# debbiemarkslab/EVcouplings

Measured on NVIDIA H100. Metric: PLM gradient evals/s as N*L^2*q cell-ops/s, higher is better.
Workload: dtype f32 parameters/accumulation; tensor-core products as bf16 hi+lo pairs (16 mantissa bits)

## Files before the change

evcouplings_b200/csrc/plm_tc.cu:

```cuda
#include <cuda.h>
#include <cuda_bf16.h>

#include <stdlib.h>

#include <algorithm>

#include "common.cuh"
#include "internal.h"

namespace evc {

constexpr int TC_BM = 128;
constexpr int TC_BN = 192;
constexpr int TC_BK = 64;
constexpr int TC_MAX_STAGES = 8;
constexpr int TC_A_BYTES = TC_BM * TC_BK * 2;
constexpr int TC_B_BYTES = TC_BN * TC_BK * 2;
constexpr int TC_SMEM_LIMIT = 232448;
constexpr int TC_SMEM_HEAD = 2048;
constexpr int TC_THREADS = 384;
constexpr int TC_CONSUMERS = 256;
constexpr int TC_K_CHUNK = 32;
constexpr int TC_MAX_KSPLIT = 8;
constexpr int TC_REG_PRODUCER = 40;
constexpr int TC_REG_CONSUMER = 232;

__device__ __forceinline__ void mbar_wait_bounded(uint64_t *bar, uint32_t parity)
{
    uint32_t done = 0;
    for (uint64_t it = 0; it < (1ull << 31); it++) {
        asm volatile(
            "{\n.reg .pred p;\n"
            "mbarrier.try_wait.parity.shared::cta.b64 p, [%1], %2;\n"
            "selp.u32 %0, 1, 0, p;\n}\n"
            : "=r"(done)
            : "r"(smem_u32(bar)), "r"(parity)
            : "memory");
        if (done) return;
    }
    __trap();
}

__device__ __forceinline__ void mbar_arrive(uint64_t *bar)
{
    asm volatile("mbarrier.arrive.shared::cta.b64 _, [%0];" ::"r"(smem_u32(bar)) : "memory");
}

__device__ __forceinline__ void tma_load_2d(void *smem_dst, const CUtensorMap *tmap, int c0, int c1, uint64_t *bar)
{
    asm volatile(
        "cp.async.bulk.tensor.2d.shared::cluster.global.mbarrier::complete_tx::bytes [%0], [%1, {%3, %4}], [%2];"
        ::"r"(smem_u32(smem_dst)), "l"(reinterpret_cast<uint64_t>(tmap)), "r"(smem_u32(bar)), "r"(c0), "r"(c1)
        : "memory");
}

__device__ __forceinline__ void tma_load_2d_hint(void *smem_dst, const CUtensorMap *tmap, int c0, int c1,
                                                 uint64_t *bar, uint64_t policy)
{
    asm volatile(
        "cp.async.bulk.tensor.2d.shared::cluster.global.mbarrier::complete_tx::bytes.L2::cache_hint "
        "[%0], [%1, {%3, %4}], [%2], %5;"
        ::"r"(smem_u32(smem_dst)), "l"(reinterpret_cast<uint64_t>(tmap)), "r"(smem_u32(bar)), "r"(c0), "r"(c1),
        "l"(policy)
        : "memory");
}
__device__ __forceinline__ uint64_t l2_policy_evict_last()
{
    uint64_t p;
    asm volatile("createpolicy.fractional.L2::evict_last.b64 %0, 1.0;" : "=l"(p));
    return p;
}

template <int N>
__device__ __forceinline__ void setmaxnreg_dec() { asm volatile("setmaxnreg.dec.sync.aligned.u32 %0;\n" ::"n"(N)); }
template <int N>
__device__ __forceinline__ void setmaxnreg_inc() { asm volatile("setmaxnreg.inc.sync.aligned.u32 %0;\n" ::"n"(N)); }

__device__ __forceinline__ void wgmma_fence() { asm volatile("wgmma.fence.sync.aligned;" ::: "memory"); }
__device__ __forceinline__ void wgmma_commit() { asm volatile("wgmma.commit_group.sync.aligned;" ::: "memory"); }
template <int N>
__device__ __forceinline__ void wgmma_wait() { asm volatile("wgmma.wait_group.sync.aligned %0;" ::"n"(N) : "memory"); }

template <int R>
__device__ __forceinline__ void fence_regs(float *d)
{
#pragma unroll
    for (int i = 0; i < R; i++) asm volatile("" : "+f"(d[i])::"memory");
}

__device__ __forceinline__ void consumer_sync() { asm volatile("bar.sync 1, %0;" ::"n"(TC_CONSUMERS) : "memory"); }

__device__ __forceinline__ uint64_t make_desc_sw128(const void *smem_ptr)
{
    const uint32_t addr = smem_u32(smem_ptr);
    uint64_t d = 0;
    d |= (uint64_t)((addr >> 4) & 0x3FFF);
    d |= (uint64_t)1 << 16;
    d |= (uint64_t)(1024 >> 4) << 32;
    d |= (uint64_t)1 << 62;
    return d;
}

template <int N>
__device__ __forceinline__ void wgmma_bf16(float *d, uint64_t da, uint64_t db, uint32_t scale_d);
template <>
__device__ __forceinline__ void wgmma_bf16<192>(float *d, uint64_t da, uint64_t db, uint32_t scale_d)
{
    asm volatile(
        "{\n.reg .pred p;\n"
        "setp.ne.b32 p, %98, 0;\n"
        "wgmma.mma_async.sync.aligned.m64n192k16.f32.bf16.bf16 "
        "{"
        "%0, %1, %2, %3, %4, %5, %6, %7, %8, %9, %10, %11, %12, %13, %14, %15, "
        "%16, %17, %18, %19, %20, %21, %22, %23, %24, %25, %26, %27, %28, %29, %30, %31, "
        "%32, %33, %34, %35, %36, %37, %38, %39, %40, %41, %42, %43, %44, %45, %46, %47, "
        "%48, %49, %50, %51, %52, %53, %54, %55, %56, %57, %58, %59, %60, %61, %62, %63, "
        "%64, %65, %66, %67, %68, %69, %70, %71, %72, %73, %74, %75, %76, %77, %78, %79, "
        "%80, %81, %82, %83, %84, %85, %86, %87, %88, %89, %90, %91, %92, %93, %94, %95"
        "}, %96, %97, p, 1, 1, 0, 0;\n}\n"
        : "+f"(d[0]), "+f"(d[1]), "+f"(d[2]), "+f"(d[3]), "+f"(d[4]), "+f"(d[5]), "+f"(d[6]), "+f"(d[7]),
          "+f"(d[8]), "+f"(d[9]), "+f"(d[10]), "+f"(d[11]), "+f"(d[12]), "+f"(d[13]), "+f"(d[14]), "+f"(d[15]),
          "+f"(d[16]), "+f"(d[17]), "+f"(d[18]), "+f"(d[19]), "+f"(d[20]), "+f"(d[21]), "+f"(d[22]), "+f"(d[23]),
          "+f"(d[24]), "+f"(d[25]), "+f"(d[26]), "+f"(d[27]), "+f"(d[28]), "+f"(d[29]), "+f"(d[30]), "+f"(d[31]),
          "+f"(d[32]), "+f"(d[33]), "+f"(d[34]), "+f"(d[35]), "+f"(d[36]), "+f"(d[37]), "+f"(d[38]), "+f"(d[39]),
          "+f"(d[40]), "+f"(d[41]), "+f"(d[42]), "+f"(d[43]), "+f"(d[44]), "+f"(d[45]), "+f"(d[46]), "+f"(d[47]),
          "+f"(d[48]), "+f"(d[49]), "+f"(d[50]), "+f"(d[51]), "+f"(d[52]), "+f"(d[53]), "+f"(d[54]), "+f"(d[55]),
          "+f"(d[56]), "+f"(d[57]), "+f"(d[58]), "+f"(d[59]), "+f"(d[60]), "+f"(d[61]), "+f"(d[62]), "+f"(d[63]),
          "+f"(d[64]), "+f"(d[65]), "+f"(d[66]), "+f"(d[67]), "+f"(d[68]), "+f"(d[69]), "+f"(d[70]), "+f"(d[71]),
          "+f"(d[72]), "+f"(d[73]), "+f"(d[74]), "+f"(d[75]), "+f"(d[76]), "+f"(d[77]), "+f"(d[78]), "+f"(d[79]),
          "+f"(d[80]), "+f"(d[81]), "+f"(d[82]), "+f"(d[83]), "+f"(d[84]), "+f"(d[85]), "+f"(d[86]), "+f"(d[87]),
          "+f"(d[88]), "+f"(d[89]), "+f"(d[90]), "+f"(d[91]), "+f"(d[92]), "+f"(d[93]), "+f"(d[94]), "+f"(d[95])
        : "l"(da), "l"(db), "r"(scale_d));
}
template <>
__device__ __forceinline__ void wgmma_bf16<176>(float *d, uint64_t da, uint64_t db, uint32_t scale_d)
{
    asm volatile(
        "{\n.reg .pred p;\n"
        "setp.ne.b32 p, %90, 0;\n"
        "wgmma.mma_async.sync.aligned.m64n176k16.f32.bf16.bf16 "
        "{"
        "%0, %1, %2, %3, %4, %5, %6, %7, %8, %9, %10, %11, %12, %13, %14, %15, "
        "%16, %17, %18, %19, %20, %21, %22, %23, %24, %25, %26, %27, %28, %29, %30, %31, "
        "%32, %33, %34, %35, %36, %37, %38, %39, %40, %41, %42, %43, %44, %45, %46, %47, "
        "%48, %49, %50, %51, %52, %53, %54, %55, %56, %57, %58, %59, %60, %61, %62, %63, "
        "%64, %65, %66, %67, %68, %69, %70, %71, %72, %73, %74, %75, %76, %77, %78, %79, "
        "%80, %81, %82, %83, %84, %85, %86, %87"
        "}, %88, %89, p, 1, 1, 0, 0;\n}\n"
        : "+f"(d[0]), "+f"(d[1]), "+f"(d[2]), "+f"(d[3]), "+f"(d[4]), "+f"(d[5]), "+f"(d[6]), "+f"(d[7]),
          "+f"(d[8]), "+f"(d[9]), "+f"(d[10]), "+f"(d[11]), "+f"(d[12]), "+f"(d[13]), "+f"(d[14]), "+f"(d[15]),
          "+f"(d[16]), "+f"(d[17]), "+f"(d[18]), "+f"(d[19]), "+f"(d[20]), "+f"(d[21]), "+f"(d[22]), "+f"(d[23]),
          "+f"(d[24]), "+f"(d[25]), "+f"(d[26]), "+f"(d[27]), "+f"(d[28]), "+f"(d[29]), "+f"(d[30]), "+f"(d[31]),
          "+f"(d[32]), "+f"(d[33]), "+f"(d[34]), "+f"(d[35]), "+f"(d[36]), "+f"(d[37]), "+f"(d[38]), "+f"(d[39]),
          "+f"(d[40]), "+f"(d[41]), "+f"(d[42]), "+f"(d[43]), "+f"(d[44]), "+f"(d[45]), "+f"(d[46]), "+f"(d[47]),
          "+f"(d[48]), "+f"(d[49]), "+f"(d[50]), "+f"(d[51]), "+f"(d[52]), "+f"(d[53]), "+f"(d[54]), "+f"(d[55]),
          "+f"(d[56]), "+f"(d[57]), "+f"(d[58]), "+f"(d[59]), "+f"(d[60]), "+f"(d[61]), "+f"(d[62]), "+f"(d[63]),
          "+f"(d[64]), "+f"(d[65]), "+f"(d[66]), "+f"(d[67]), "+f"(d[68]), "+f"(d[69]), "+f"(d[70]), "+f"(d[71]),
          "+f"(d[72]), "+f"(d[73]), "+f"(d[74]), "+f"(d[75]), "+f"(d[76]), "+f"(d[77]), "+f"(d[78]), "+f"(d[79]),
          "+f"(d[80]), "+f"(d[81]), "+f"(d[82]), "+f"(d[83]), "+f"(d[84]), "+f"(d[85]), "+f"(d[86]), "+f"(d[87])
        : "l"(da), "l"(db), "r"(scale_d));
}

__device__ __forceinline__ void wgmma_sp_bf16_192(float *d, const uint4 &a, uint32_t e, uint64_t db, uint32_t scale_d)
{
    asm volatile(
        "{\n.reg .pred p;\n"
        "setp.ne.b32 p, %102, 0;\n"
        "wgmma.mma_async.sp.sync.aligned.m64n192k32.f32.bf16.bf16 "
        "{"
        "%0, %1, %2, %3, %4, %5, %6, %7, %8, %9, %10, %11, %12, %13, %14, %15, "
        "%16, %17, %18, %19, %20, %21, %22, %23, %24, %25, %26, %27, %28, %29, %30, %31, "
        "%32, %33, %34, %35, %36, %37, %38, %39, %40, %41, %42, %43, %44, %45, %46, %47, "
        "%48, %49, %50, %51, %52, %53, %54, %55, %56, %57, %58, %59, %60, %61, %62, %63, "
        "%64, %65, %66, %67, %68, %69, %70, %71, %72, %73, %74, %75, %76, %77, %78, %79, "
        "%80, %81, %82, %83, %84, %85, %86, %87, %88, %89, %90, %91, %92, %93, %94, %95"
        "}, {%96, %97, %98, %99}, %100, %101, 0, p, 1, 1, 0;\n}\n"
        : "+f"(d[0]), "+f"(d[1]), "+f"(d[2]), "+f"(d[3]), "+f"(d[4]), "+f"(d[5]), "+f"(d[6]), "+f"(d[7]),
          "+f"(d[8]), "+f"(d[9]), "+f"(d[10]), "+f"(d[11]), "+f"(d[12]), "+f"(d[13]), "+f"(d[14]), "+f"(d[15]),
// ... 54 lines not shown
                                             bool overwrite)
{
#pragma unroll
    for (int k = 0; k < TC_BK / 16; k++) {
        const uint64_t koff = (uint64_t)((k * 16 * 2) >> 4);
        wgmma_bf16<N>(acc, a + koff, b + koff, (overwrite && k == 0) ? 0u : 1u);
        if (two) wgmma_bf16<N>(acc, a2 + koff, b2 + koff, 1u);
    }
}

template <int N>
__device__ __forceinline__ void tc_mainloop(float *acc, uint64_t *full, uint64_t *empty, int &s, uint32_t &ph,
                                            int n_stages, int stage_bytes, int kb0, int kb1, uint64_t desc0,
                                            uint64_t off_a, uint64_t off_b, uint64_t off_a2, uint64_t off_b2, bool two)
{
    int prev = -1;
    for (int kb = kb0; kb < kb1; kb++) {
        mbar_wait_bounded(&full[s], ph);
        wgmma_fence();
        const uint64_t d = desc0 + (uint64_t)((s * stage_bytes) >> 4);
        wgmma_kblock<N>(acc, d + off_a, d + off_b, d + off_a2, d + off_b2, two, kb == kb0);
        wgmma_commit();
        wgmma_wait<1>();
        if (prev >= 0) mbar_arrive(&empty[prev]);
        prev = s;
        if (++s == n_stages) { s = 0; ph ^= 1u; }
    }
    wgmma_wait<0>();
    fence_regs<N / 2>(acc);
    if (prev >= 0) mbar_arrive(&empty[prev]);
}

__device__ __forceinline__ void decode_tile(int tile, int m_tiles, int n_tiles, int mgroup, int &m_tile, int &n_tile)
{
    const int full = (m_tiles / mgroup) * mgroup * n_tiles;
    if (tile < full) {
        const int per = mgroup * n_tiles;
        const int g = tile / per, r = tile - g * per;
        n_tile = r / mgroup;
        m_tile = g * mgroup + (r - n_tile * mgroup);
    } else {
        const int rem = m_tiles % mgroup, r = tile - full;
        n_tile = r / rem;
        m_tile = (m_tiles / mgroup) * mgroup + (r - n_tile * rem);
    }
}

struct TcSmem {
    uint64_t *full, *empty;
    unsigned char *ring;
};
__device__ __forceinline__ TcSmem tc_smem_layout(unsigned char *smem_dyn)
{
    unsigned char *base = reinterpret_cast<unsigned char *>((reinterpret_cast<uintptr_t>(smem_dyn) + 1023) &
                                                            ~static_cast<uintptr_t>(1023));
    TcSmem l;
    l.full = reinterpret_cast<uint64_t *>(base);
    l.empty = l.full + TC_MAX_STAGES;
    l.ring = base + 1024;
    return l;
}
__device__ __forceinline__ void tc_init_barriers(const TcSmem &l, int n_stages)
{
    if (threadIdx.x == 0) {
        for (int s = 0; s < n_stages; s++) {
            mbar_init(&l.full[s], 1);
            mbar_init(&l.empty[s], TC_CONSUMERS);
        }
        mbar_fence_init();
    }
    __syncthreads();
}

template <int SINGLE, int ACC = 0>
__global__ void __launch_bounds__(TC_THREADS, 1)
tc_gemm_kernel(const __grid_constant__ CUtensorMap tm0, const __grid_constant__ CUtensorMap tm1,
               const __grid_constant__ CUtensorMap tm2, float *__restrict__ D, int64_t ldd, int m_tiles, int n_tiles,
               int num_kb, int k_chunk, int mgroup, int n_stages, int ksplit, int64_t plane, int acc_planes)
{
    constexpr int BYTES0 = TC_A_BYTES;
    constexpr int BYTES1 = TC_B_BYTES;
    constexpr int BYTES2 = TC_B_BYTES;
    constexpr int stage_bytes = BYTES0 + BYTES1 + (SINGLE ? 0 : BYTES2);
    extern __shared__ unsigned char smem_dyn[];
    const TcSmem l = tc_smem_layout(smem_dyn);
    const int tiles = m_tiles * n_tiles;
    const int slice = (int)blockIdx.x / tiles;
    int m_tile, n_tile;
    decode_tile((int)blockIdx.x - slice * tiles, m_tiles, n_tiles, mgroup, m_tile, n_tile);
    const int kb_per = (num_kb + ksplit - 1) / ksplit;
    const int kb_begin = slice * kb_per, kb_end = min(num_kb, kb_begin + kb_per);
    tc_init_barriers(l, n_stages);

    if (threadIdx.x < 128) {
        setmaxnreg_dec<TC_REG_PRODUCER>();
        if (threadIdx.x == 0) {
            int s = 0;
            uint32_t ph = 0;
            for (int kb = kb_begin; kb < kb_end; kb++) {
                mbar_wait_bounded(&l.empty[s], ph ^ 1u);
                unsigned char *st = l.ring + s * stage_bytes;
                mbar_expect_tx(&l.full[s], (uint32_t)stage_bytes);
                tma_load_2d(st, &tm0, kb * TC_BK, m_tile * TC_BM, &l.full[s]);
                tma_load_2d(st + BYTES0, &tm1, kb * TC_BK, n_tile * TC_BN, &l.full[s]);
                if (!SINGLE) tma_load_2d(st + BYTES0 + BYTES1, &tm2, kb * TC_BK, n_tile * TC_BN, &l.full[s]);
                if (++s == n_stages) { s = 0; ph ^= 1u; }
            }
        }
    } else {
        setmaxnreg_inc<TC_REG_CONSUMER>();
        const int cw = (threadIdx.x >> 7) - 1;
        constexpr uint64_t OFF1 = (uint64_t)(BYTES0 >> 4), OFF2 = (uint64_t)((BYTES0 + BYTES1) >> 4);
        const uint64_t arow = (uint64_t)((cw * 64 * TC_BK * 2) >> 4);
        const uint64_t desc0 = make_desc_sw128(l.ring);
        float acc[TC_BN / 2], sum[TC_BN / 2];
#pragma unroll
        for (int u = 0; u < TC_BN / 2; u++) acc[u] = 0.f;
        const int n_chunks = (kb_end - kb_begin + k_chunk - 1) / k_chunk;
        int s = 0;
        uint32_t ph = 0;
        for (int c = 0; c < n_chunks; c++) {
            const int kb0 = kb_begin + c * k_chunk, kb1 = min(kb_end, kb0 + k_chunk);
            tc_mainloop<TC_BN>(acc, l.full, l.empty, s, ph, n_stages, stage_bytes, kb0, kb1, desc0,
                               arow, OFF1, arow, OFF2, !SINGLE);
#pragma unroll
            for (int u = 0; u < TC_BN / 2; u++) sum[u] = (c == 0) ? acc[u] : sum[u] + acc[u];
        }
        const int t = threadIdx.x & 127;
        const int64_t row = (int64_t)m_tile * TC_BM + cw * 64 + (t >> 5) * 16 + ((t & 31) >> 2);
        float *out = D + slice * plane + row * ldd + (int64_t)n_tile * TC_BN + 2 * (t & 3);
        if (ACC && slice < acc_planes) {
#pragma unroll
            for (int c8 = 0; c8 < TC_BN / 8; c8++) {
                float2 *p0 = reinterpret_cast<float2 *>(out + 8 * c8);
                float2 *p1 = reinterpret_cast<float2 *>(out + 8 * ldd + 8 * c8);
                const float2 v0 = __ldcs(p0), v1 = __ldcs(p1);
                __stcs(p0, make_float2(v0.x + sum[4 * c8], v0.y + sum[4 * c8 + 1]));
                __stcs(p1, make_float2(v1.x + sum[4 * c8 + 2], v1.y + sum[4 * c8 + 3]));
            }
            return;
        }
#pragma unroll
        for (int c8 = 0; c8 < TC_BN / 8; c8++) {
            __stcs(reinterpret_cast<float2 *>(out + 8 * c8), make_float2(sum[4 * c8], sum[4 * c8 + 1]));
            __stcs(reinterpret_cast<float2 *>(out + 8 * ldd + 8 * c8), make_float2(sum[4 * c8 + 2], sum[4 * c8 + 3]));
        }
    }
}

constexpr int XSP_STEP_BYTES = 2560;
constexpr int XSP_KB_BYTES = 4 * XSP_STEP_BYTES;
constexpr int SP_W_HALF = (TC_BN / 2) * TC_BK * 2;

template <int SINGLE>
__global__ void __launch_bounds__(TC_THREADS, 1)
tc_sparse_logits_kernel(const __grid_constant__ CUtensorMap tm_hi, const __grid_constant__ CUtensorMap tm_lo,
                        const unsigned char *__restrict__ xsp, float *__restrict__ Zt, int64_t ldz, int64_t rows_z,
                        int state_tiles, int seq_tiles, int seq_units, int num_kb, int k_chunk, int group,
                        int n_stages)
{
    constexpr int OFF_A = TC_B_BYTES;
    constexpr int OFF_LO = TC_B_BYTES + XSP_KB_BYTES;
    constexpr int stage_bytes = OFF_LO + (SINGLE ? 0 : TC_B_BYTES);
    extern __shared__ unsigned char smem_dyn[];
    const TcSmem l = tc_smem_layout(smem_dyn);
    uint32_t cs;
    asm volatile("mov.u32 %0, %%cluster_nctarank;" : "=r"(cs));
    const uint32_t rank = cluster_ctarank();
    int n_tile, unit;
    decode_tile((int)(blockIdx.x / cs), state_tiles, seq_units, group, n_tile, unit);
    const int seq_tile = unit * (int)cs + (int)rank;
    const bool pad = seq_tile >= seq_tiles;
    if (threadIdx.x == 0) {
        for (int s = 0; s < n_stages; s++) {
            mbar_init(&l.full[s], 1);
            mbar_init(&l.empty[s], 8 * cs);
        }
        mbar_fence_init();
    }
    cluster_sync();

    if (threadIdx.x < 128) {
        setmaxnreg_dec<TC_REG_PRODUCER>();
        if (threadIdx.x == 0) {
            const uint64_t keep = l2_policy_evict_last();
            const unsigned char *src = xsp + (int64_t)(pad ? 0 : seq_tile) * num_kb * XSP_KB_BYTES;
            const int row0 = n_tile * TC_BN;
            int s = 0;
            uint32_t ph = 0;
            for (int kb = 0; kb < num_kb; kb++) {
                mbar_wait_bounded(&l.empty[s], ph ^ 1u);
                unsigned char *st = l.ring + s * stage_bytes;
                mbar_expect_tx(&l.full[s], (uint32_t)stage_bytes);
                bulk_g2s(st + OFF_A, src + (int64_t)kb * XSP_KB_BYTES, XSP_KB_BYTES, &l.full[s]);
                if (cs == 1) {
                    for (int h = 0; h < 2; h++) {
                        tma_load_2d_hint(st + h * SP_W_HALF, &tm_hi, kb * TC_BK, row0 + h * (TC_BN / 2), &l.full[s], keep);
                        if (!SINGLE)
                            tma_load_2d_hint(st + OFF_LO + h * SP_W_HALF, &tm_lo, kb * TC_BK, row0 + h * (TC_BN / 2),
                                             &l.full[s], keep);
                    }
                } else {
                    const int h = (int)rank;
                    tma_load_2d_multicast(st + h * SP_W_HALF, &tm_hi, kb * TC_BK, row0 + h * (TC_BN / 2), &l.full[s],
                                          (uint16_t)0x3, keep);
                    if (!SINGLE)
                        tma_load_2d_multicast(st + OFF_LO + h * SP_W_HALF, &tm_lo, kb * TC_BK, row0 + h * (TC_BN / 2),
                                              &l.full[s], (uint16_t)0x3, keep);
                }
                if (++s == n_stages) { s = 0; ph ^= 1u; }
            }
        }
    } else {
        setmaxnreg_inc<TC_REG_CONSUMER>();
        const int cw = (threadIdx.x >> 7) - 1;
        const int t = threadIdx.x & 127;
        const uint32_t a_addr = smem_u32(l.ring) + OFF_A + cw * 2 * XSP_STEP_BYTES + 16 * t;
        const uint32_t e_addr = a_addr + 2048 - 12 * t;
        const uint64_t desc0 = make_desc_sw128(l.ring);
        constexpr uint64_t DLO = (uint64_t)(OFF_LO >> 4), DK32 = (uint64_t)((32 * 2) >> 4);
        auto release = [&](int st) {
            if ((threadIdx.x & 31) == 0) {
                mbar_arrive_cluster(&l.empty[st], 0);
                if (cs == 2) mbar_arrive_cluster(&l.empty[st], 1);
            }
        };
        float acc[TC_BN / 2], sum[TC_BN / 2];
#pragma unroll
        for (int u = 0; u < TC_BN / 2; u++) acc[u] = 0.f;
        const int n_chunks = (num_kb + k_chunk - 1) / k_chunk;
        int s = 0;
        uint32_t ph = 0;
        for (int c = 0; c < n_chunks; c++) {
            const int kb0 = c * k_chunk, kb1 = min(num_kb, kb0 + k_chunk);
            for (int kb = kb0; kb < kb1; kb++) {
                mbar_wait_bounded(&l.full[s], ph);
                const uint32_t so = (uint32_t)(s * stage_bytes);
                const uint4 a0 = lds128(a_addr + so), a1 = lds128(a_addr + so + XSP_STEP_BYTES);
                const uint32_t e0 = lds32(e_addr + so), e1 = lds32(e_addr + so + XSP_STEP_BYTES);
                wgmma_fence();
                const uint64_t d = desc0 + (uint64_t)((s * stage_bytes) >> 4);
                wgmma_sp_bf16_192(acc, a0, e0, d, kb == kb0 ? 0u : 1u);
                if (!SINGLE) wgmma_sp_bf16_192(acc, a0, e0, d + DLO, 1u);
                wgmma_sp_bf16_192(acc, a1, e1, d + DK32, 1u);
                if (!SINGLE) wgmma_sp_bf16_192(acc, a1, e1, d + DLO + DK32, 1u);
                wgmma_commit();
                wgmma_wait<0>();
                release(s);
                if (++s == n_stages) { s = 0; ph ^= 1u; }
            }
            fence_regs<TC_BN / 2>(acc);
#pragma unroll
            for (int u = 0; u < TC_BN / 2; u++) sum[u] = (c == 0) ? acc[u] : sum[u] + acc[u];
        }
        if (!pad) {
            const int64_t seq0 = (int64_t)seq_tile * TC_BM + cw * 64 + (t >> 5) * 16 + ((t & 31) >> 2);
            const int64_t st0 = (int64_t)n_tile * TC_BN + 2 * (t & 3);
#pragma unroll
            for (int c8 = 0; c8 < TC_BN / 8; c8++)
#pragma unroll
                for (int e = 0; e < 4; e++) {
                    const int64_t row = st0 + 8 * c8 + (e & 1), col = seq0 + 8 * (e >> 1);
                    if (row < rows_z && col < ldz) __stcs(Zt + row * ldz + col, sum[4 * c8 + e]);
                }
        }
    }
    cluster_sync();
}

__device__ __forceinline__ uint32_t xsp_group(const uint32_t *__restrict__ msa4, int64_t Nld, int64_t n, bool real,
                                              int k, int lq, int q, uint32_t &vals)
{
    uint32_t mask = 0;
    if (real) {
#pragma unroll
        for (int p = 0; p < 4; p++) {
            const int kk = k + p;
            if (kk >= lq) break;
            const int j = kk / q, b = kk - j * q;
            const int code = (int)((msa4[(int64_t)(j >> 2) * Nld + n] >> (8 * (j & 3))) & 0xffu);
            mask |= (uint32_t)(code == b) << p;
        }
    }
    int i0 = 0, i1 = 1;
    if (__popc(mask) == 2) { i0 = __ffs(mask) - 1; i1 = 31 - __clz(mask); }
    else if (mask > 2) i1 = __ffs(mask) - 1;
    vals = (((mask >> i0) & 1u) ? 0x3F80u : 0u) | ((((mask >> i1) & 1u) ? 0x3F80u : 0u) << 16);
    return (uint32_t)(i0 | (i1 << 2));
}

__global__ void build_xsp_kernel(const uint32_t *__restrict__ msa4, unsigned char *__restrict__ out, int64_t n0,
                                 int64_t nreal, int64_t Nld, int L, int q, int num_kb, int64_t n_frag)
{
    const int64_t gt = (int64_t)blockIdx.x * blockDim.x + threadIdx.x;
    if (gt >= n_frag * 128) return;
    const int64_t ci = gt >> 7;
    const int t = (int)(gt & 127);
    const int step = (int)(ci & 1), cw = (int)((ci >> 1) & 1);
    const int64_t tkb = ci >> 2;
    const int kb = (int)(tkb % num_kb);
    const int64_t T = tkb / num_kb;
    const int64_t r0 = T * TC_BM + cw * 64 + (t >> 5) * 16 + ((t & 31) >> 2), r1 = r0 + 8;
    const int k0 = kb * TC_BK + step * 32, lq = L * q;
    const int c = t & 3, h = c & 1;
    uint32_t e = 0, v[2][2], unused;
#pragma unroll
    for (int rr = 0; rr < 2; rr++) {
        const int64_t r = rr ? r1 : r0;
#pragma unroll
        for (int i = 0; i < 4; i++)
            e |= xsp_group(msa4, Nld, n0 + r, r < nreal, k0 + 4 * (4 * h + i), lq, q, unused) << (16 * rr + 4 * i);
#pragma unroll
        for (int u = 0; u < 2; u++) xsp_group(msa4, Nld, n0 + r, r < nreal, k0 + 4 * (4 * u + c), lq, q, v[rr][u]);
    }
    unsigned char *frag = out + ci * XSP_STEP_BYTES;
    reinterpret_cast<uint4 *>(frag)[t] = make_uint4(v[0][0], v[1][0], v[0][1], v[1][1]);
    reinterpret_cast<uint32_t *>(frag + 2048)[t] = e;
}

constexpr int TF_BN = 176;
constexpr int TF_SITES = 8;
constexpr int TF_B_BYTES = TF_BN * TC_BK * 2;
constexpr int TF_PITCH = TF_BN + 1;

template <int SINGLE>
__global__ void __launch_bounds__(TC_THREADS, 1)
tc_fwd_fused_kernel(const __grid_constant__ CUtensorMap tm_x, const __grid_constant__ CUtensorMap tm_whi,
                    const __grid_constant__ CUtensorMap tm_wlo, const float *__restrict__ h,
                    const uint32_t *__restrict__ msa4, const float *__restrict__ wts,
                    __nv_bfloat16 *__restrict__ Rt_hi, __nv_bfloat16 *__restrict__ Rt_lo, int64_t Kp,
                    float *__restrict__ gh_part, double *__restrict__ fx_part, PlmGeom g, int m_tiles, int n_tiles,
                    int num_kb, int n_stages)
{
    constexpr int Q = 21;
    extern __shared__ unsigned char smem_dyn[];
    const TcSmem l = tc_smem_layout(smem_dyn);
    constexpr int stage_bytes = TC_A_BYTES + TF_B_BYTES + (SINGLE ? 0 : TF_B_BYTES);
    const int n_tile = blockIdx.x % n_tiles, m_tile = blockIdx.x / n_tiles;
    const int q = g.q;
    tc_init_barriers(l, n_stages);

    if (threadIdx.x < 128) {
        setmaxnreg_dec<TC_REG_PRODUCER>();
        if (threadIdx.x == 0) {
            const uint64_t keep = l2_policy_evict_last();
            int s = 0;
            uint32_t ph = 0;
            for (int kb = 0; kb < num_kb; kb++) {
                mbar_wait_bounded(&l.empty[s], ph ^ 1u);
                unsigned char *st = l.ring + s * stage_bytes;
                mbar_expect_tx(&l.full[s], (uint32_t)stage_bytes);
                tma_load_2d(st, &tm_x, kb * TC_BK, m_tile * TC_BM, &l.full[s]);
                tma_load_2d_hint(st + TC_A_BYTES, &tm_whi, kb * TC_BK, n_tile * TF_BN, &l.full[s], keep);
                if (!SINGLE)
                    tma_load_2d_hint(st + TC_A_BYTES + TF_B_BYTES, &tm_wlo, kb * TC_BK, n_tile * TF_BN, &l.full[s], keep);
                if (++s == n_stages) { s = 0; ph ^= 1u; }
            }
        }
        return;
    }
    setmaxnreg_inc<TC_REG_CONSUMER>();
    const int ct = threadIdx.x - 128;
    {
        const int cw = ct >> 7;
        const uint64_t arow = (uint64_t)((cw * 64 * TC_BK * 2) >> 4);
        constexpr uint64_t OFFH = (uint64_t)(TC_A_BYTES >> 4), OFFL = (uint64_t)((TC_A_BYTES + TF_B_BYTES) >> 4);
        float acc[TF_BN / 2];
#pragma unroll
        for (int u = 0; u < TF_BN / 2; u++) acc[u] = 0.f;
        int s = 0;
        uint32_t ph = 0;
        tc_mainloop<TF_BN>(acc, l.full, l.empty, s, ph, n_stages, stage_bytes, 0, num_kb, make_desc_sw128(l.ring),
                           arow, OFFH, arow, OFFL, !SINGLE);
        consumer_sync();
        float *stg = reinterpret_cast<float *>(l.ring);
        const int t = ct & 127;
        const int r0 = cw * 64 + (t >> 5) * 16 + ((t & 31) >> 2);
#pragma unroll
        for (int c8 = 0; c8 < TF_BN / 8; c8++) {
            const int col = 8 * c8 + 2 * (t & 3);
            stg[r0 * TF_PITCH + col] = acc[4 * c8];
            stg[r0 * TF_PITCH + col + 1] = acc[4 * c8 + 1];
            stg[(r0 + 8) * TF_PITCH + col] = acc[4 * c8 + 2];
            stg[(r0 + 8) * TF_PITCH + col + 1] = acc[4 * c8 + 3];
        }
        consumer_sync();
    }
    const float *stg = reinterpret_cast<const float *>(l.ring);
    const int ehalf = ct >> 7;
    const int r = ct & 127;
    const int quad = r >> 5, lane = r & 31;
    const int ntile_part = m_tiles * 4;
    const int64_t n = (int64_t)m_tile * TC_BM + r;
    const int64_t nc = n < g.N ? n : g.N - 1;
    const float wn = n < g.N ? wts[nc] : 0.f;
    const float *v = stg + r * TF_PITCH + ehalf * 88;
#pragma unroll
    for (int s = 0; s < 4; s++) {
        const int i = n_tile * TF_SITES + ehalf * 4 + s;
        if (i >= g.L) break;
        const int si = (int)((msa4[(int64_t)(i >> 2) * g.Nld + nc] >> (8 * (i & 3))) & 0xffu);
        const float w = si < q ? wn : 0.f;
        float z[Q];
        float mx = -INFINITY;
#pragma unroll
        for (int a = 0; a < Q; a++) {
            z[a] = (a < q) ? v[s * Q + a] + h[i * q + a] : -INFINITY;
            mx = fmaxf(mx, z[a]);
        }
        float zs = 0.f, sum = 0.f;
#pragma unroll
        for (int a = 0; a < Q; a++) {
            if (a == si) zs = z[a];
            z[a] = (a < q) ? expf(z[a] - mx) : 0.f;
            sum += z[a];
        }
        const double fx_local = (w == 0.f) ? 0.0 : -((double)w * (double)(zs - mx - logf(sum)));
// ... 383 lines not shown
{
    dim3 grid((unsigned)ceil_div(t.Kp, 256), (unsigned)g.L);
    build_xt_kernel<<<grid, 256, 0, st>>>(d_msa4, reinterpret_cast<__nv_bfloat16 *>(d_xt), n0, g.N, g.Nld, t.Kp,
                                          g.L, g.q);
    EVC_KERNEL_CHECK();
    return 0;
}

int plm_tc_make_maps(const PlmTcGeom &t, void *d_xt, void *d_rt_hi, void *d_rt_lo, void *maps_out)
{
    CUtensorMap *m = reinterpret_cast<CUtensorMap *>(maps_out);
    if (make_map(&m[0], d_xt, t.Mp, t.Kp, TC_BM)) return 1;
    if (make_map(&m[1], d_rt_hi, t.Np, t.Kp, TC_BN)) return 1;
    if (make_map(&m[2], d_rt_lo, t.Np, t.Kp, TC_BN)) return 1;
    return 0;
}

int plm_tc_backward(const PlmGeom &g, const PlmTcGeom &t, const void *maps, float *d_Gd, int single, int chunk,
                    cudaStream_t st)
{
    const CUtensorMap *m = reinterpret_cast<const CUtensorMap *>(maps);
    const int stage = TC_A_BYTES + TC_B_BYTES + (single ? 0 : TC_B_BYTES);
    const int n_stages = stages_for(stage);
    const size_t smem = (size_t)n_stages * stage + TC_SMEM_HEAD;
    static int kc_env = -2;
    const int kc = env_int_once("EVC_KCHUNK", &kc_env);
    const int k_chunk = kc > 0 ? kc : TC_K_CHUNK;
    const int m_tiles = (int)(t.Mp / TC_BM), n_tiles = (int)(t.Np / TC_BN);
    const bool last = chunk == t.n_chunks - 1;
    const int ksplit = last ? t.ksplit_last : t.ksplit;
    const int num_kb = (int)(t.kp_chunk(chunk, g.N) / TC_BK);
    const int grid = m_tiles * n_tiles * ksplit;
    const int64_t plane = t.Mp * t.Np;
    if (chunk == 0) {
        if (single) {
            EVC_CUDA(cudaFuncSetAttribute(tc_gemm_kernel<1>, cudaFuncAttributeMaxDynamicSharedMemorySize, TC_SMEM_LIMIT));
            tc_gemm_kernel<1><<<grid, TC_THREADS, smem, st>>>(m[0], m[1], m[2], d_Gd, t.Np, m_tiles, n_tiles,
                                                                num_kb, k_chunk, m_tiles, n_stages, ksplit, plane, 0);
        } else {
            EVC_CUDA(cudaFuncSetAttribute(tc_gemm_kernel<0>, cudaFuncAttributeMaxDynamicSharedMemorySize, TC_SMEM_LIMIT));
            tc_gemm_kernel<0><<<grid, TC_THREADS, smem, st>>>(m[0], m[1], m[2], d_Gd, t.Np, m_tiles, n_tiles,
                                                                num_kb, k_chunk, m_tiles, n_stages, ksplit, plane, 0);
        }
    } else {
        const int acc_planes = t.ksplit;
        if (single) {
            EVC_CUDA(cudaFuncSetAttribute(tc_gemm_kernel<1, 1>, cudaFuncAttributeMaxDynamicSharedMemorySize, TC_SMEM_LIMIT));
            tc_gemm_kernel<1, 1><<<grid, TC_THREADS, smem, st>>>(m[0], m[1], m[2], d_Gd, t.Np, m_tiles, n_tiles,
                                                                   num_kb, k_chunk, m_tiles, n_stages, ksplit, plane,
                                                                   acc_planes);
        } else {
            EVC_CUDA(cudaFuncSetAttribute(tc_gemm_kernel<0, 1>, cudaFuncAttributeMaxDynamicSharedMemorySize, TC_SMEM_LIMIT));
            tc_gemm_kernel<0, 1><<<grid, TC_THREADS, smem, st>>>(m[0], m[1], m[2], d_Gd, t.Np, m_tiles, n_tiles,
                                                                   num_kb, k_chunk, m_tiles, n_stages, ksplit, plane,
                                                                   acc_planes);
        }
    }
    EVC_KERNEL_CHECK();
    return 0;
}

int plm_tc_finalize_pairs(const PlmGeom &g, const PlmTcGeom &t, const float *d_Gd, int planes, float *d_gJ,
                          float scale, cudaStream_t st)
{
    const unsigned nt = (unsigned)ceil_div(g.L, FIN_SITES);
    auto kernel = g.q > 21 ? finalize_pairs_tc_kernel<true> : finalize_pairs_tc_kernel<false>;
    const int smem = fin_smem_bytes(g.q);
    EVC_CUDA(cudaFuncSetAttribute(kernel, cudaFuncAttributeMaxDynamicSharedMemorySize, smem));
    kernel<<<dim3(nt, nt), FIN_THREADS, smem, st>>>(d_Gd, planes, t.Mp * t.Np, d_gJ, g.L, g.q, (int)t.Np, scale,
                                                    fin_pitch(g.q));
    EVC_KERNEL_CHECK();
    return 0;
}

void plm_tcf_geometry(const PlmGeom &g, const PlmTcGeom &tc, PlmTcfGeom &t)
{
    const int64_t lq = (int64_t)g.L * g.q;
    t.Mp = round_up(lq, TC_BM);
    t.Kw = round_up(lq, TC_BK);
    t.Ns = round_up(tc.C, TC_BN);
    t.Xrows = round_up(tc.C, 384);
    t.ntiles_s = (int)ceil_div(g.N, 256);
}

int plm_tcf_build_x(const PlmGeom &g, const PlmTcfGeom &t, const uint32_t *d_msa4, void *d_x1h, int64_t n0,
                    cudaStream_t st)
{
    build_x_kernel<<<(unsigned)t.Xrows, 256, 0, st>>>(d_msa4, reinterpret_cast<__nv_bfloat16 *>(d_x1h), n0,
                                                    std::min(t.Xrows, g.N - n0), g.Nld, g.L, g.q, t.Kw);
    EVC_KERNEL_CHECK();
    return 0;
}

int plm_tcf_make_maps(const PlmTcfGeom &t, void *d_wt_hi, void *d_wt_lo, void *maps_out)
{
    CUtensorMap *m = reinterpret_cast<CUtensorMap *>(maps_out);
    if (make_map(&m[0], d_wt_hi, t.Mp, t.Kw, TC_BN / 2)) return 1;
    if (make_map(&m[1], d_wt_lo, t.Mp, t.Kw, TC_BN / 2)) return 1;
    return 0;
}

int plm_tcf_build_xsp(const PlmGeom &g, const PlmTcfGeom &t, const uint32_t *d_msa4, void *d_x1h, int64_t n0,
                      cudaStream_t st)
{
    const int num_kb = (int)(t.Kw / TC_BK);
    const int64_t n_frag = t.Xrows / TC_BM * num_kb * 4;
    build_xsp_kernel<<<(unsigned)ceil_div(n_frag * 128, 256), 256, 0, st>>>(
        d_msa4, reinterpret_cast<unsigned char *>(d_x1h), n0, std::min(t.Xrows, g.N - n0), g.Nld, g.L, g.q, num_kb,
        n_frag);
    EVC_KERNEL_CHECK();
    return 0;
}

int plm_tcf_expand(const PlmGeom &g, const PlmTcfGeom &t, const float *d_x, void *d_wt_hi, void *d_wt_lo,
                   int single, cudaStream_t st)
{
    const unsigned nt = (unsigned)ceil_div(g.L, EXP_SITES);
    if (g.q > EXP_STATIC_Q) {
        const size_t smem = exp_wide_smem(g.q);
        EVC_CUDA(cudaFuncSetAttribute(expand_tc_kernel<false, true>, cudaFuncAttributeMaxDynamicSharedMemorySize,
                                      (int)smem));
        expand_tc_kernel<false, true><<<dim3(nt, nt), EXP_THREADS, smem, st>>>(
            d_x, reinterpret_cast<__nv_bfloat16 *>(d_wt_hi), reinterpret_cast<__nv_bfloat16 *>(d_wt_lo), g.L, g.q,
            t.Kw, single);
        EVC_KERNEL_CHECK();
        return 0;
    }
    expand_tc_kernel<false><<<dim3(nt, nt), EXP_THREADS, 0, st>>>(d_x, reinterpret_cast<__nv_bfloat16 *>(d_wt_hi),
                                                                  reinterpret_cast<__nv_bfloat16 *>(d_wt_lo), g.L, g.q,
                                                                  t.Kw, single);
    EVC_KERNEL_CHECK();
    return 0;
}

static int forward_group(const PlmTcfGeom &t, int single, int tiles)
{
    static int mg_env = -2;
    const int e = env_int_once("EVC_MGROUP", &mg_env);
    if (e > 0) return std::min(e, tiles);
    static int mb_env = -2;
    const int mb = env_int_once("EVC_MGROUP_MB", &mb_env);
    const double budget = (mb > 0 ? mb : 24) * 1.0e6;
    const double per_tile = (double)TC_BN * (double)t.Kw * 2.0 * (single ? 1.0 : 2.0);
    return std::max(1, std::min(tiles, (int)(budget / per_tile)));
}

static int forward_cluster()
{
    static int cl_env = -2;
    const int e = env_int_once("EVC_FWD_CLUSTER", &cl_env);
    return e == 1 ? 1 : 2;
}

int plm_tcf_logits(const PlmGeom &g, const PlmTcfGeom &t, const void *maps, const void *d_x1h, float *d_zt,
                   int single, int64_t nreal, cudaStream_t st)
{
    const CUtensorMap *m = reinterpret_cast<const CUtensorMap *>(maps);
    const int stage = TC_B_BYTES + XSP_KB_BYTES + (single ? 0 : TC_B_BYTES);
    const int n_stages = stages_for(stage);
    const size_t smem = (size_t)n_stages * stage + TC_SMEM_HEAD;
    const int cs = forward_cluster();
    const int state_tiles = (int)ceil_div((int64_t)g.L * g.q, TC_BN);
    const int seq_tiles = (int)ceil_div(nreal, TC_BM), seq_units = (int)ceil_div(seq_tiles, cs);
    const int num_kb = (int)(t.Kw / TC_BK);
    const int kchunk = num_kb <= 128 ? num_kb : TC_K_CHUNK;
    const int group = forward_group(t, single, state_tiles);
    auto kernel = single ? tc_sparse_logits_kernel<1> : tc_sparse_logits_kernel<0>;
    EVC_CUDA(cudaFuncSetAttribute(kernel, cudaFuncAttributeMaxDynamicSharedMemorySize, TC_SMEM_LIMIT));
    cudaLaunchConfig_t cfg = {};
    cfg.gridDim = dim3((unsigned)(state_tiles * seq_units * cs));
    cfg.blockDim = dim3(TC_THREADS);
    cfg.dynamicSmemBytes = smem;
    cfg.stream = st;
    cudaLaunchAttribute attr[1];
    attr[0].id = cudaLaunchAttributeClusterDimension;
    attr[0].val.clusterDim.x = (unsigned)cs;
    attr[0].val.clusterDim.y = 1;
    attr[0].val.clusterDim.z = 1;
    cfg.attrs = attr;
    cfg.numAttrs = 1;
    EVC_CUDA(cudaLaunchKernelEx(&cfg, kernel, m[0], m[1], reinterpret_cast<const unsigned char *>(d_x1h), d_zt, t.Ns,
                                t.Mp, state_tiles, seq_tiles, seq_units, num_kb, kchunk, group, n_stages));
    EVC_KERNEL_CHECK();
    return 0;
}

template <bool ONEHOT>
static int launch_softmax(const PlmGeom &g, int ntiles, const float *d_zt, int64_t ldz, const float *d_x,
                          const uint32_t *d_msa4, const float *d_wts, __nv_bfloat16 *hi, __nv_bfloat16 *lo,
                          int64_t Kp, float *d_gh_part, double *d_fx_part, int64_t n0, int64_t nreal, cudaStream_t st)
{
    dim3 grid((unsigned)ceil_div(nreal, 256), (unsigned)g.L);
    switch (g.q) {
        case 21: plm_softmax_kernel<21, ONEHOT><<<grid, 128, 0, st>>>(d_zt, ldz, d_x, d_msa4, d_wts, hi, lo, Kp, d_gh_part, d_fx_part, g, ntiles, n0); break;
        case 20: plm_softmax_kernel<20, ONEHOT><<<grid, 128, 0, st>>>(d_zt, ldz, d_x, d_msa4, d_wts, hi, lo, Kp, d_gh_part, d_fx_part, g, ntiles, n0); break;
        case 5: plm_softmax_kernel<5, ONEHOT><<<grid, 128, 0, st>>>(d_zt, ldz, d_x, d_msa4, d_wts, hi, lo, Kp, d_gh_part, d_fx_part, g, ntiles, n0); break;
        case 4: plm_softmax_kernel<4, ONEHOT><<<grid, 128, 0, st>>>(d_zt, ldz, d_x, d_msa4, d_wts, hi, lo, Kp, d_gh_part, d_fx_part, g, ntiles, n0); break;
        default:
            if (g.q < 2 || g.q > PLM_MAX_Q) { set_error("plm softmax kernel: unsupported q"); return 1; }
            if (g.q <= 8)
                plm_softmax_kernel<8, ONEHOT, true><<<grid, 128, 0, st>>>(d_zt, ldz, d_x, d_msa4, d_wts, hi, lo, Kp, d_gh_part, d_fx_part, g, ntiles, n0);
            else if (g.q <= 16)
                plm_softmax_kernel<16, ONEHOT, true><<<grid, 128, 0, st>>>(d_zt, ldz, d_x, d_msa4, d_wts, hi, lo, Kp, d_gh_part, d_fx_part, g, ntiles, n0);
            else
                plm_softmax_kernel<32, ONEHOT, true><<<grid, 128, 0, st>>>(d_zt, ldz, d_x, d_msa4, d_wts, hi, lo, Kp, d_gh_part, d_fx_part, g, ntiles, n0);
    }
    EVC_KERNEL_CHECK();
    return 0;
}

int plm_tcf_softmax(const PlmGeom &g, const PlmTcfGeom &t, const float *d_zt, const float *d_x,
                    const uint32_t *d_msa4, const float *d_wts, void *d_rt_hi, void *d_rt_lo, int64_t Kp,
                    float *d_gh_part, double *d_fx_part, int64_t n0, int64_t nreal, cudaStream_t st)
{
    return launch_softmax<false>(g, t.ntiles_s, d_zt, t.Ns, d_x, d_msa4, d_wts,
                                 reinterpret_cast<__nv_bfloat16 *>(d_rt_hi), reinterpret_cast<__nv_bfloat16 *>(d_rt_lo),
                                 Kp, d_gh_part, d_fx_part, n0, nreal, st);
}

int plm_tc_onehot_residual(const PlmGeom &g, int ntiles, const uint32_t *d_msa4, const float *d_wts, void *d_rt_hi,
                           void *d_rt_lo, int64_t Kp, float *d_gh_part, double *d_fx_part, int64_t n0, int64_t nreal,
                           cudaStream_t st)
{
    return launch_softmax<true>(g, ntiles, nullptr, 0, nullptr, d_msa4, d_wts,
                                reinterpret_cast<__nv_bfloat16 *>(d_rt_hi), reinterpret_cast<__nv_bfloat16 *>(d_rt_lo),
                                Kp, d_gh_part, d_fx_part, n0, nreal, st);
}

void plm_tcff_geometry(const PlmGeom &g, PlmTcffGeom &t)
{
    t.n_tiles = (int)ceil_div(g.L, TF_SITES);
    t.Np = (int64_t)t.n_tiles * TF_BN;
    t.Kw = round_up((int64_t)g.L * g.q, TC_BK);
    t.m_tiles = (int)ceil_div(g.N, TC_BM);
    t.Xrows = round_up(g.N, 384);
    t.ntile_part = t.m_tiles * 4;
}

bool plm_tcff_supported(const PlmGeom &g) { return g.S == 21; }

int plm_tcff_make_maps(const PlmTcffGeom &t, void *d_x1h, void *d_wp_hi, void *d_wp_lo, void *maps_out)
{
    CUtensorMap *m = reinterpret_cast<CUtensorMap *>(maps_out);
    if (make_map(&m[0], d_x1h, t.Xrows, t.Kw, TC_BM)) return 1;
    if (make_map(&m[1], d_wp_hi, t.Np, t.Kw, TF_BN)) return 1;
    if (make_map(&m[2], d_wp_lo, t.Np, t.Kw, TF_BN)) return 1;
    return 0;
}

int plm_tcff_expand(const PlmGeom &g, const PlmTcffGeom &t, const float *d_x, void *d_wp_hi, void *d_wp_lo,
                    int single, cudaStream_t st)
{
    const unsigned nt = (unsigned)ceil_div(g.L, EXP_SITES);
    expand_tc_kernel<true><<<dim3(nt, nt), EXP_THREADS, 0, st>>>(d_x, reinterpret_cast<__nv_bfloat16 *>(d_wp_hi),
                                                                 reinterpret_cast<__nv_bfloat16 *>(d_wp_lo), g.L, g.q,
                                                                 t.Kw, single);
    EVC_KERNEL_CHECK();
    return 0;
}

int plm_tcff_forward(const PlmGeom &g, const PlmTcffGeom &t, const void *maps, const float *d_x,
                     const uint32_t *d_msa4, const float *d_wts, void *d_rt_hi, void *d_rt_lo, int64_t Kp,
                     float *d_gh_part, double *d_fx_part, int single, cudaStream_t st)
{
    const CUtensorMap *m = reinterpret_cast<const CUtensorMap *>(maps);
    const int stage = TC_A_BYTES + TF_B_BYTES + (single ? 0 : TF_B_BYTES);
    const int n_stages = stages_for(stage);
    const size_t smem = (size_t)n_stages * stage + TC_SMEM_HEAD;
    const int grid = t.m_tiles * t.n_tiles;
    auto kernel = single ? tc_fwd_fused_kernel<1> : tc_fwd_fused_kernel<0>;
    EVC_CUDA(cudaFuncSetAttribute(kernel, cudaFuncAttributeMaxDynamicSharedMemorySize, TC_SMEM_LIMIT));
    kernel<<<grid, TC_THREADS, smem, st>>>(m[0], m[1], m[2], d_x, d_msa4, d_wts, reinterpret_cast<__nv_bfloat16 *>(d_rt_hi),
                                           reinterpret_cast<__nv_bfloat16 *>(d_rt_lo), Kp, d_gh_part, d_fx_part, g,
                                           t.m_tiles, t.n_tiles, (int)(t.Kw / TC_BK), n_stages);
    EVC_KERNEL_CHECK();
    return 0;
}

size_t plm_tc_map_bytes() { return 3 * sizeof(CUtensorMap); }

}
```

Baseline: 4798 billion.

## Process two sequence tiles per CTA in sparse logits kernel to reuse weight loads

Adds a PAIR variant of the sparse-logits wgmma kernel in which each consumer warpgroup holds two accumulators and covers two 128-row sequence tiles, so each TMA-loaded weight tile feeds twice as many MMAs. This halves weight traffic per output and halves the grid size. Register budgets are rebalanced toward consumers (240/24) to fit the doubled accumulators. The variant is used by default when there is no K chunking, and it raises stage size (fewer pipeline stages) and register-spill risk.

```diff
diff --git a/evcouplings_b200/csrc/plm_tc.cu b/evcouplings_b200/csrc/plm_tc.cu
--- a/evcouplings_b200/csrc/plm_tc.cu
+++ b/evcouplings_b200/csrc/plm_tc.cu
@@ -24,6 +24,8 @@
 constexpr int TC_MAX_KSPLIT = 8;
 constexpr int TC_REG_PRODUCER = 40;
 constexpr int TC_REG_CONSUMER = 232;
+constexpr int TC_REG_PRODUCER_PAIR = 24;
+constexpr int TC_REG_CONSUMER_PAIR = 240;
 
 __device__ __forceinline__ void mbar_wait_bounded(uint64_t *bar, uint32_t parity)
 {
@@ -384,15 +386,16 @@
 constexpr int XSP_KB_BYTES = 4 * XSP_STEP_BYTES;
 constexpr int SP_W_HALF = (TC_BN / 2) * TC_BK * 2;
 
-template <int SINGLE>
+template <int SINGLE, int PAIR>
 __global__ void __launch_bounds__(TC_THREADS, 1)
 tc_sparse_logits_kernel(const __grid_constant__ CUtensorMap tm_hi, const __grid_constant__ CUtensorMap tm_lo,
                         const unsigned char *__restrict__ xsp, float *__restrict__ Zt, int64_t ldz, int64_t rows_z,
                         int state_tiles, int seq_tiles, int seq_units, int num_kb, int k_chunk, int group,
                         int n_stages)
 {
+    constexpr int TILES = PAIR ? 2 : 1;
     constexpr int OFF_A = TC_B_BYTES;
-    constexpr int OFF_LO = TC_B_BYTES + XSP_KB_BYTES;
+    constexpr int OFF_LO = TC_B_BYTES + TILES * XSP_KB_BYTES;
     constexpr int stage_bytes = OFF_LO + (SINGLE ? 0 : TC_B_BYTES);
     extern __shared__ unsigned char smem_dyn[];
     const TcSmem l = tc_smem_layout(smem_dyn);
@@ -401,8 +404,7 @@
     const uint32_t rank = cluster_ctarank();
     int n_tile, unit;
     decode_tile((int)(blockIdx.x / cs), state_tiles, seq_units, group, n_tile, unit);
-    const int seq_tile = unit * (int)cs + (int)rank;
-    const bool pad = seq_tile >= seq_tiles;
+    const int seq_tile0 = (unit * (int)cs + (int)rank) * TILES;
     if (threadIdx.x == 0) {
         for (int s = 0; s < n_stages; s++) {
             mbar_init(&l.full[s], 1);
@@ -413,10 +415,15 @@
     cluster_sync();
 
     if (threadIdx.x < 128) {
-        setmaxnreg_dec<TC_REG_PRODUCER>();
+        setmaxnreg_dec<PAIR ? TC_REG_PRODUCER_PAIR : TC_REG_PRODUCER>();
         if (threadIdx.x == 0) {
             const uint64_t keep = l2_policy_evict_last();
-            const unsigned char *src = xsp + (int64_t)(pad ? 0 : seq_tile) * num_kb * XSP_KB_BYTES;
+            const unsigned char *src[TILES];
+#pragma unroll
+            for (int i = 0; i < TILES; i++) {
+                const int tile = seq_tile0 + i;
+                src[i] = xsp + (int64_t)(tile >= seq_tiles ? 0 : tile) * num_kb * XSP_KB_BYTES;
+            }
             const int row0 = n_tile * TC_BN;
             int s = 0;
             uint32_t ph = 0;
@@ -424,7 +431,10 @@
                 mbar_wait_bounded(&l.empty[s], ph ^ 1u);
                 unsigned char *st = l.ring + s * stage_bytes;
                 mbar_expect_tx(&l.full[s], (uint32_t)stage_bytes);
-                bulk_g2s(st + OFF_A, src + (int64_t)kb * XSP_KB_BYTES, XSP_KB_BYTES, &l.full[s]);
+#pragma unroll
+                for (int i = 0; i < TILES; i++)
+                    bulk_g2s(st + OFF_A + i * XSP_KB_BYTES, src[i] + (int64_t)kb * XSP_KB_BYTES, XSP_KB_BYTES,
+                             &l.full[s]);
                 if (cs == 1) {
                     for (int h = 0; h < 2; h++) {
                         tma_load_2d_hint(st + h * SP_W_HALF, &tm_hi, kb * TC_BK, row0 + h * (TC_BN / 2), &l.full[s], keep);
@@ -444,10 +454,10 @@
             }
         }
     } else {
-        setmaxnreg_inc<TC_REG_CONSUMER>();
+        setmaxnreg_inc<PAIR ? TC_REG_CONSUMER_PAIR : TC_REG_CONSUMER>();
         const int cw = (threadIdx.x >> 7) - 1;
         const int t = threadIdx.x & 127;
-        const uint32_t a_addr = smem_u32(l.ring) + OFF_A + cw * 2 * XSP_STEP_BYTES + 16 * t;
+        const uint32_t a_addr = smem_u32(l.ring) + OFF_A + cw * (PAIR ? XSP_KB_BYTES : 2 * XSP_STEP_BYTES) + 16 * t;
         const uint32_t e_addr = a_addr + 2048 - 12 * t;
         const uint64_t desc0 = make_desc_sw128(l.ring);
         constexpr uint64_t DLO = (uint64_t)(OFF_LO >> 4), DK32 = (uint64_t)((32 * 2) >> 4);
@@ -457,44 +467,96 @@
                 if (cs == 2) mbar_arrive_cluster(&l.empty[st], 1);
             }
         };
-        float acc[TC_BN / 2], sum[TC_BN / 2];
-#pragma unroll
-        for (int u = 0; u < TC_BN / 2; u++) acc[u] = 0.f;
-        const int n_chunks = (num_kb + k_chunk - 1) / k_chunk;
-        int s = 0;
-        uint32_t ph = 0;
-        for (int c = 0; c < n_chunks; c++) {
-            const int kb0 = c * k_chunk, kb1 = min(num_kb, kb0 + k_chunk);
-            for (int kb = kb0; kb < kb1; kb++) {
+        auto store = [&](const float *const *v, int nb, int tile, int rb) {
+            if (tile >= seq_tiles) return;
+            const int64_t seq0 = (int64_t)tile * TC_BM + rb + (t >> 5) * 16 + ((t & 31) >> 2);
+            const int64_t st0 = (int64_t)n_tile * TC_BN + 2 * (t & 3);
+            bool col[2][2];
+#pragma unroll
+            for (int b = 0; b < 2; b++)
+#pragma unroll
+                for (int h = 0; h < 2; h++) col[b][h] = b < nb && seq0 + 64 * b + 8 * h < ldz;
+            const int64_t nrows = rows_z - st0;
+            float *p = Zt + st0 * ldz + seq0;
+#pragma unroll
+            for (int c8 = 0; c8 < TC_BN / 8; c8++) {
+#pragma unroll
+                for (int e = 0; e < 4; e++)
+#pragma unroll
+                    for (int b = 0; b < 2; b++)
+                        if (8 * c8 + (e & 1) < nrows && col[b][e >> 1])
+                            __stcs(p + (e & 1) * ldz + 64 * b + 8 * (e >> 1), v[b][4 * c8 + e]);
+                p += 8 * ldz;
+            }
+        };
+        if (PAIR) {
+            float acc0[TC_BN / 2], acc1[TC_BN / 2];
+#pragma unroll
+            for (int u = 0; u < TC_BN / 2; u++) acc0[u] = acc1[u] = 0.f;
+            int s = 0;
+            uint32_t ph = 0;
+            for (int kb = 0; kb < num_kb; kb++) {
                 mbar_wait_bounded(&l.full[s], ph);
                 const uint32_t so = (uint32_t)(s * stage_bytes);
-                const uint4 a0 = lds128(a_addr + so), a1 = lds128(a_addr + so + XSP_STEP_BYTES);
-                const uint32_t e0 = lds32(e_addr + so), e1 = lds32(e_addr + so + XSP_STEP_BYTES);
+                const uint4 a00 = lds128(a_addr + so), a01 = lds128(a_addr + so + XSP_STEP_BYTES);
+                const uint4 a10 = lds128(a_addr + so + 2 * XSP_STEP_BYTES), a11 = lds128(a_addr + so + 3 * XSP_STEP_BYTES);
+                const uint32_t e00 = lds32(e_addr + so), e01 = lds32(e_addr + so + XSP_STEP_BYTES);
+                const uint32_t e10 = lds32(e_addr + so + 2 * XSP_STEP_BYTES), e11 = lds32(e_addr + so + 3 * XSP_STEP_BYTES);
                 wgmma_fence();
                 const uint64_t d = desc0 + (uint64_t)((s * stage_bytes) >> 4);
-                wgmma_sp_bf16_192(acc, a0, e0, d, kb == kb0 ? 0u : 1u);
-                if (!SINGLE) wgmma_sp_bf16_192(acc, a0, e0, d + DLO, 1u);
-                wgmma_sp_bf16_192(acc, a1, e1, d + DK32, 1u);
-                if (!SINGLE) wgmma_sp_bf16_192(acc, a1, e1, d + DLO + DK32, 1u);
+                const uint32_t sc = kb == 0 ? 0u : 1u;
+                wgmma_sp_bf16_192(acc0, a00, e00, d, sc);
+                wgmma_sp_bf16_192(acc1, a10, e10, d, sc);
+                if (!SINGLE) {
+                    wgmma_sp_bf16_192(acc0, a00, e00, d + DLO, 1u);
+                    wgmma_sp_bf16_192(acc1, a10, e10, d + DLO, 1u);
+                }
+                wgmma_sp_bf16_192(acc0, a01, e01, d + DK32, 1u);
+                wgmma_sp_bf16_192(acc1, a11, e11, d + DK32, 1u);
+                if (!SINGLE) {
+                    wgmma_sp_bf16_192(acc0, a01, e01, d + DLO + DK32, 1u);
+                    wgmma_sp_bf16_192(acc1, a11, e11, d + DLO + DK32, 1u);
+                }
                 wgmma_commit();
                 wgmma_wait<0>();
                 release(s);
                 if (++s == n_stages) { s = 0; ph ^= 1u; }
             }
-            fence_regs<TC_BN / 2>(acc);
-#pragma unroll
-            for (int u = 0; u < TC_BN / 2; u++) sum[u] = (c == 0) ? acc[u] : sum[u] + acc[u];
-        }
-        if (!pad) {
-            const int64_t seq0 = (int64_t)seq_tile * TC_BM + cw * 64 + (t >> 5) * 16 + ((t & 31) >> 2);
-            const int64_t st0 = (int64_t)n_tile * TC_BN + 2 * (t & 3);
-#pragma unroll
-            for (int c8 = 0; c8 < TC_BN / 8; c8++)
-#pragma unroll
-                for (int e = 0; e < 4; e++) {
-                    const int64_t row = st0 + 8 * c8 + (e & 1), col = seq0 + 8 * (e >> 1);
-                    if (row < rows_z && col < ldz) __stcs(Zt + row * ldz + col, sum[4 * c8 + e]);
+            fence_regs<TC_BN / 2>(acc0);
+            fence_regs<TC_BN / 2>(acc1);
+            const float *v[2] = {acc0, acc1};
+            store(v, 2, seq_tile0 + cw, 0);
+        } else {
+            float acc[TC_BN / 2], sum[TC_BN / 2];
+#pragma unroll
+            for (int u = 0; u < TC_BN / 2; u++) acc[u] = 0.f;
+            const int n_chunks = (num_kb + k_chunk - 1) / k_chunk;
+            int s = 0;
+            uint32_t ph = 0;
+            for (int c = 0; c < n_chunks; c++) {
+                const int kb0 = c * k_chunk, kb1 = min(num_kb, kb0 + k_chunk);
+                for (int kb = kb0; kb < kb1; kb++) {
+                    mbar_wait_bounded(&l.full[s], ph);
+                    const uint32_t so = (uint32_t)(s * stage_bytes);
+                    const uint4 a0 = lds128(a_addr + so), a1 = lds128(a_addr + so + XSP_STEP_BYTES);
+                    const uint32_t e0 = lds32(e_addr + so), e1 = lds32(e_addr + so + XSP_STEP_BYTES);
+                    wgmma_fence();
+                    const uint64_t d = desc0 + (uint64_t)((s * stage_bytes) >> 4);
+                    wgmma_sp_bf16_192(acc, a0, e0, d, kb == kb0 ? 0u : 1u);
+                    if (!SINGLE) wgmma_sp_bf16_192(acc, a0, e0, d + DLO, 1u);
+                    wgmma_sp_bf16_192(acc, a1, e1, d + DK32, 1u);
+                    if (!SINGLE) wgmma_sp_bf16_192(acc, a1, e1, d + DLO + DK32, 1u);
+                    wgmma_commit();
+                    wgmma_wait<0>();
+                    release(s);
+                    if (++s == n_stages) { s = 0; ph ^= 1u; }
                 }
+                fence_regs<TC_BN / 2>(acc);
+#pragma unroll
+                for (int u = 0; u < TC_BN / 2; u++) sum[u] = (c == 0) ? acc[u] : sum[u] + acc[u];
+            }
+            const float *v[2] = {sum, sum};
+            store(v, 1, seq_tile0, cw * 64);
         }
     }
     cluster_sync();
@@ -1184,20 +1246,30 @@
     return e == 1 ? 1 : 2;
 }
 
+static bool forward_pair(int num_kb, int kchunk)
+{
+    static int tile_env = -2;
+    const int e = env_int_once("EVC_FWD_TILE", &tile_env);
+    return e != 128 && kchunk >= num_kb;
+}
+
 int plm_tcf_logits(const PlmGeom &g, const PlmTcfGeom &t, const void *maps, const void *d_x1h, float *d_zt,
                    int single, int64_t nreal, cudaStream_t st)
 {
     const CUtensorMap *m = reinterpret_cast<const CUtensorMap *>(maps);
-    const int stage = TC_B_BYTES + XSP_KB_BYTES + (single ? 0 : TC_B_BYTES);
+    const int num_kb = (int)(t.Kw / TC_BK);
+    const int kchunk = num_kb <= 128 ? num_kb : TC_K_CHUNK;
+    const bool pair = forward_pair(num_kb, kchunk);
+    const int stage = TC_B_BYTES + (pair ? 2 : 1) * XSP_KB_BYTES + (single ? 0 : TC_B_BYTES);
     const int n_stages = stages_for(stage);
     const size_t smem = (size_t)n_stages * stage + TC_SMEM_HEAD;
     const int cs = forward_cluster();
     const int state_tiles = (int)ceil_div((int64_t)g.L * g.q, TC_BN);
-    const int seq_tiles = (int)ceil_div(nreal, TC_BM), seq_units = (int)ceil_div(seq_tiles, cs);
-    const int num_kb = (int)(t.Kw / TC_BK);
-    const int kchunk = num_kb <= 128 ? num_kb : TC_K_CHUNK;
+    const int seq_tiles = (int)ceil_div(nreal, TC_BM);
+    const int seq_units = (int)ceil_div(ceil_div(seq_tiles, pair ? 2 : 1), cs);
     const int group = forward_group(t, single, state_tiles);
-    auto kernel = single ? tc_sparse_logits_kernel<1> : tc_sparse_logits_kernel<0>;
+    auto kernel = pair ? (single ? tc_sparse_logits_kernel<1, 1> : tc_sparse_logits_kernel<0, 1>)
+                       : (single ? tc_sparse_logits_kernel<1, 0> : tc_sparse_logits_kernel<0, 0>);
     EVC_CUDA(cudaFuncSetAttribute(kernel, cudaFuncAttributeMaxDynamicSharedMemorySize, TC_SMEM_LIMIT));
     cudaLaunchConfig_t cfg = {};
     cfg.gridDim = dim3((unsigned)(state_tiles * seq_units * cs));
```

After: 5098 billion, median of 6. +6.2%, better.
